# sanazkaviani/3d-latent-diffusion-model

Hardware: AMD Instinct MI355X
Metric: UNet denoising steps/sec (bf16, 1x4x24x24x24 latent; whole job = sum over GPUs) (higher is better)
Workload: dtype bf16

## Files before the change

3d-latent-diffusion-model_amd/csrc/attention.h:

```cpp
#pragma once
#include "common.h"

struct AttnParams {
    const bf16_t* qkv; bf16_t* out;
    int B, N, C, heads; float scale;
    float* lse;
    int d;
};

template <int S, int QW, bool DB, int D = 64>
__global__ __launch_bounds__(64 * QW * S) void attn_fwd_kernel(const AttnParams p) {
    constexpr int KT = 64;
    constexpr int NSL = (D + 63) / 64, DS = D < 64 ? D : 64;
    constexpr int K2 = DS / 32, NDT = DS / 16, CH = DS / 8;
    constexpr int IMG = KT * 128;
    constexpr int TILE = 2 * NSL * IMG;
    constexpr int GT = 64 * QW;
    constexpr int NIT = (KT * CH * NSL) / GT;
    static_assert(S == 1 || D == 64, "the in-workgroup key split is built for D = 64");
    static_assert((KT * CH * NSL) % GT == 0, "staging must divide evenly");
    extern __shared__ __attribute__((aligned(16))) char smem_all[];

    const int tid = threadIdx.x % GT, lane = tid & 63, wave = tid >> 6, grp = threadIdx.x / GT;
    char* smem = smem_all + grp * (DB ? 2 : 1) * TILE;
    const int fr = lane & 15, fg = lane >> 4;
    const int b = blockIdx.z, head = blockIdx.y;
    const int q0 = blockIdx.x * (16 * QW) + wave * 16;
    const int ld = 3 * p.C;
    const bf16_t* base = p.qkv + (size_t)b * p.N * ld;
    const int hoff = head * D;

    bf16x8 qf[NSL][K2];
    {
        int qr = q0 + fr; if (qr >= p.N) qr = p.N - 1;
#pragma unroll
        for (int sl = 0; sl < NSL; ++sl)
#pragma unroll
            for (int k2 = 0; k2 < K2; ++k2)
                qf[sl][k2] = *reinterpret_cast<const bf16x8*>(base + (size_t)qr * ld + hoff + sl * 64 + k2 * 32 + 8 * fg);
    }

    f32x4 ot[NSL][NDT];
#pragma unroll
    for (int sl = 0; sl < NSL; ++sl)
#pragma unroll
        for (int i = 0; i < NDT; ++i) ot[sl][i] = (f32x4){0.f, 0.f, 0.f, 0.f};
    float mrun = -INFINITY, lrun = 0.f;
    const float cexp = p.scale * 1.44269504088896340736f;

    u32x4 kreg[NIT], vreg[NIT];
    auto stage_load = [&](int k0) {
#pragma unroll
        for (int it = 0; it < NIT; ++it) {
            const int idx = tid + it * GT;
            const int sl = idx / (KT * CH), rem = idx - sl * (KT * CH);
            const int row = rem / CH, ch = rem - row * CH;
            int kr = k0 + row; if (kr >= p.N) kr = p.N - 1;
            const bf16_t* tok = base + (size_t)kr * ld + hoff + sl * 64 + ch * 8;
            kreg[it] = *reinterpret_cast<const u32x4*>(tok + p.C);
            vreg[it] = *reinterpret_cast<const u32x4*>(tok + 2 * p.C);
        }
    };
    auto stage_write = [&](char* ks, char* vs) {
#pragma unroll
        for (int it = 0; it < NIT; ++it) {
            const int idx = tid + it * GT;
            const int sl = idx / (KT * CH), rem = idx - sl * (KT * CH);
            const int row = rem / CH, ch = rem - row * CH;
            *reinterpret_cast<u32x4*>(ks + sl * IMG + row * 128 + ((ch ^ ((row >> 1) & 7)) << 4)) = kreg[it];
            *reinterpret_cast<u32x4*>(vs + sl * IMG + row * 128 + ((ch ^ (((row >> 1) & 3) << 1)) << 4)) = vreg[it];
        }
    };

    const int ntile = (p.N + KT - 1) / KT;
    const int nrounds = (ntile + S - 1) / S;
    stage_load(grp * KT);
#pragma unroll
    for (int sl = 0; sl < NSL; ++sl)
#pragma unroll
        for (int k2 = 0; k2 < K2; ++k2) asm volatile("" :: "v"(qf[sl][k2]));
    stage_write(smem, smem + NSL * IMG);
    __syncthreads();
    for (int it = 0; it < nrounds; ++it) {
        const int t = it * S + grp;
        const int k0 = t * KT;
        const char* ks = smem + (DB ? (it & 1) * TILE : 0);
        const char* vs = ks + NSL * IMG;
        stage_load(k0 + S * KT);
        if (t < ntile) {
        f32x4 st[4];
#pragma unroll
        for (int j = 0; j < 4; ++j) {
            st[j] = (f32x4){0.f, 0.f, 0.f, 0.f};
            const int row = j * 16 + fr;
#pragma unroll
            for (int sl = 0; sl < NSL; ++sl)
#pragma unroll
                for (int k2 = 0; k2 < K2; ++k2) {
                    const int c = k2 * 4 + fg;
                    const bf16x8 kf = *reinterpret_cast<const bf16x8*>(ks + sl * IMG + row * 128 + ((c ^ ((row >> 1) & 7)) << 4));
                    st[j] = __builtin_amdgcn_mfma_f32_16x16x32_bf16(kf, qf[sl][k2], st[j], 0, 0, 0);
                }
        }
        if (k0 + KT > p.N) {
#pragma unroll
            for (int j = 0; j < 4; ++j)
#pragma unroll
                for (int r = 0; r < 4; ++r)
                    if (k0 + 16 * j + 4 * fg + r >= p.N) st[j][r] = -INFINITY;
        }
        float tmax = fmaxf(fmaxf(fmaxf(st[0][0], st[0][1]), fmaxf(st[0][2], st[0][3])), fmaxf(fmaxf(st[1][0], st[1][1]), fmaxf(st[1][2], st[1][3])));
        tmax = fmaxf(tmax, fmaxf(fmaxf(fmaxf(st[2][0], st[2][1]), fmaxf(st[2][2], st[2][3])), fmaxf(fmaxf(st[3][0], st[3][1]), fmaxf(st[3][2], st[3][3]))));
        tmax = fmaxf(tmax, __shfl_xor(tmax, 16, 64));
        tmax = fmaxf(tmax, __shfl_xor(tmax, 32, 64));
        const float mnew = fmaxf(mrun, tmax);
        const float alpha = __builtin_amdgcn_exp2f((mrun - mnew) * cexp);
        const float mc = -mnew * cexp;
        mrun = mnew;
        float psum = 0.f;
        bf16x8 pf[2];
#pragma unroll
        for (int h = 0; h < 2; ++h) {
            float pv[8];
#pragma unroll
            for (int e = 0; e < 8; ++e) {
                const float pe = __builtin_amdgcn_exp2f(fmaf(st[2 * h + (e >> 2)][e & 3], cexp, mc));
                psum += pe;
                pv[e] = pe;
            }
            u32x4 pk;
#pragma unroll
            for (int e = 0; e < 4; ++e) pk[e] = pack2bf(pv[2 * e], pv[2 * e + 1]);
            pf[h] = *reinterpret_cast<bf16x8*>(&pk);
        }
        lrun = lrun * alpha + psum;
        if (__builtin_amdgcn_ballot_w64(alpha != 1.0f)) {
#pragma unroll
            for (int sl = 0; sl < NSL; ++sl)
#pragma unroll
                for (int dt = 0; dt < NDT; ++dt) {
#pragma unroll
                    for (int r = 0; r < 4; ++r) ot[sl][dt][r] *= alpha;
                }
        }
        typedef __attribute__((ext_vector_type(4))) short s16x4;
        typedef __attribute__((address_space(3))) s16x4* lds_s16x4_t;
        const int tq = fr >> 2, tp = fr & 3;
#pragma unroll
        for (int sl = 0; sl < NSL; ++sl)
#pragma unroll
        for (int dt = 0; dt < NDT; ++dt) {
#pragma unroll
            for (int h = 0; h < 2; ++h) {
                const int rlo = (2 * h) * 16 + 4 * fg + tq, rhi = rlo + 16;
                const char* alo = vs + sl * IMG + rlo * 128 + ((dt ^ ((rlo >> 1) & 3)) << 5) + tp * 8;
                const char* ahi = vs + sl * IMG + rhi * 128 + ((dt ^ ((rhi >> 1) & 3)) << 5) + tp * 8;
                const s16x4 lo = __builtin_amdgcn_ds_read_tr16_b64_v4i16((lds_s16x4_t)alo);
                const s16x4 hi = __builtin_amdgcn_ds_read_tr16_b64_v4i16((lds_s16x4_t)ahi);
                const bf16x8 vf = {lo[0], lo[1], lo[2], lo[3], hi[0], hi[1], hi[2], hi[3]};
                ot[sl][dt] = __builtin_amdgcn_mfma_f32_16x16x32_bf16(vf, pf[h], ot[sl][dt], 0, 0, 0);
            }
        }
        }
        if constexpr (!DB) __syncthreads();
        {
            char* nk = smem + (DB ? ((it + 1) & 1) * TILE : 0);
            stage_write(nk, nk + NSL * IMG);
        }
        __syncthreads();
    }
    lrun += __shfl_xor(lrun, 16, 64);
    lrun += __shfl_xor(lrun, 32, 64);
    if constexpr (S > 1) {
        float* xo = reinterpret_cast<float*>(smem_all) + (size_t)(grp * QW + wave) * (1024 + 32);
        if (grp > 0) {
#pragma unroll
            for (int dt = 0; dt < NDT; ++dt) *reinterpret_cast<f32x4*>(xo + (dt * 64 + lane) * 4) = ot[0][dt];
            if (fg == 0) { xo[1024 + fr] = mrun; xo[1040 + fr] = lrun; }
        }
        __syncthreads();
        if (grp > 0) return;
#pragma unroll
        for (int g = 1; g < S; ++g) {
            const float* xg = reinterpret_cast<const float*>(smem_all) + (size_t)(g * QW + wave) * (1024 + 32);
            const float mg = xg[1024 + fr], lg = xg[1040 + fr];
            const float mnew = fmaxf(mrun, mg);
            const float a0 = __builtin_amdgcn_exp2f((mrun - mnew) * cexp), a1 = __builtin_amdgcn_exp2f((mg - mnew) * cexp);
            lrun = lrun * a0 + lg * a1;
            mrun = mnew;
#pragma unroll
            for (int dt = 0; dt < NDT; ++dt) {
                const f32x4 og = *reinterpret_cast<const f32x4*>(xg + (dt * 64 + lane) * 4);
#pragma unroll
                for (int r = 0; r < 4; ++r) ot[0][dt][r] = ot[0][dt][r] * a0 + og[r] * a1;
            }
        }
    }
    const float inv = 1.0f / lrun;
    const int qr = q0 + fr;
    if (p.lse && qr < p.N && fg == 0) p.lse[((size_t)b * p.heads + head) * p.N + qr] = mrun * p.scale + __logf(lrun);
    if (qr < p.N) {
        bf16_t* orow = p.out + ((size_t)b * p.N + qr) * p.C + hoff;
#pragma unroll
        for (int sl = 0; sl < NSL; ++sl)
#pragma unroll
        for (int dt = 0; dt < NDT; ++dt) {
            u32x2 o;
            o[0] = pack2bf(ot[sl][dt][0] * inv, ot[sl][dt][1] * inv);
            o[1] = pack2bf(ot[sl][dt][2] * inv, ot[sl][dt][3] * inv);
            *reinterpret_cast<u32x2*>(orow + sl * 64 + dt * 16 + 4 * fg) = o;
        }
    }
}

template <int D>
static inline hipError_t launch_attn_fwd_d(const AttnParams& p, hipStream_t s) {
    constexpr int LDS = 2 * 2 * ((D + 63) / 64) * 64 * 128;
    static bool once_tab[32] = {}; bool& once = attr_flag(once_tab);
    if (!once) {
        hipError_t e = hipFuncSetAttribute(reinterpret_cast<const void*>(&attn_fwd_kernel<1, 4, true, D>), hipFuncAttributeMaxDynamicSharedMemorySize, LDS);
        if (e != hipSuccess) return e;
        once = true;
    }
    hipLaunchKernelGGL((attn_fwd_kernel<1, 4, true, D>), dim3((p.N + 63) / 64, p.heads, p.B), dim3(256), LDS, s, p);
    return hipGetLastError();
}
static inline hipError_t launch_attn_fwd(const AttnParams& p, hipStream_t s) {
    if (p.d == 32) return launch_attn_fwd_d<32>(p, s);
    if (p.d == 128) return launch_attn_fwd_d<128>(p, s);
    if (p.d == 256) return launch_attn_fwd_d<256>(p, s);
    if (p.d != 64) return hipErrorInvalidValue;
    static bool once_tab[32] = {}; bool& once = attr_flag(once_tab);
    if (!once) {
        hipError_t e = hipFuncSetAttribute(reinterpret_cast<const void*>(&attn_fwd_kernel<4, 4, true>), hipFuncAttributeMaxDynamicSharedMemorySize, 4 * 32768);
        if (e == hipSuccess) e = hipFuncSetAttribute(reinterpret_cast<const void*>(&attn_fwd_kernel<8, 2, false>), hipFuncAttributeMaxDynamicSharedMemorySize, 8 * 16384);
        if (e != hipSuccess) return e;
        once = true;
    }
    if (p.N >= 1024 && (long)((p.N + 63) / 64) * p.heads * p.B < 128)
        hipLaunchKernelGGL((attn_fwd_kernel<8, 2, false>), dim3((p.N + 31) / 32, p.heads, p.B), dim3(1024), 8 * 16384, s, p);
    else if (p.N > 3 * 64) hipLaunchKernelGGL((attn_fwd_kernel<4, 4, true>), dim3((p.N + 63) / 64, p.heads, p.B), dim3(1024), 4 * 32768, s, p);
    else hipLaunchKernelGGL((attn_fwd_kernel<1, 4, true>), dim3((p.N + 63) / 64, p.heads, p.B), dim3(256), 32768, s, p);
    return hipGetLastError();
}


struct AttnBwdParams {
    const bf16_t* qkv; const bf16_t* o; const bf16_t* d_o; const float* lse;
    float* delta;
    bf16_t* dqkv;
    int B, N, C, heads; float scale;
    int d;
};

__global__ __launch_bounds__(256) void attn_delta_kernel(const AttnBwdParams p) {
    const long idx = (long)blockIdx.x * 256 + threadIdx.x;
    const int cpd = p.d >> 3;
    const long total = (long)p.B * p.N * p.heads * cpd;
    float s = 0.f;
    long tok = 0; int head = 0;
    if (idx < total) {
        const int ch = (int)(idx % cpd);
        const long th = idx / cpd;
        head = (int)(th % p.heads); tok = th / p.heads;
        const u32x4 a = *reinterpret_cast<const u32x4*>(p.o + tok * p.C + head * p.d + ch * 8);
        const u32x4 b = *reinterpret_cast<const u32x4*>(p.d_o + tok * p.C + head * p.d + ch * 8);
#pragma unroll
        for (int k = 0; k < 4; ++k)
            s += __uint_as_float(a[k] << 16) * __uint_as_float(b[k] << 16) +
                 __uint_as_float(a[k] & 0xffff0000u) * __uint_as_float(b[k] & 0xffff0000u);
    }
    for (int o = 1; o < cpd; o <<= 1) s += __shfl_xor(s, o, 64);
    if (idx < total && (idx % cpd) == 0) {
        const long bb = tok / p.N, i = tok - bb * p.N;
        p.delta[((size_t)bb * p.heads + head) * p.N + i] = s;
    }
}

typedef __attribute__((ext_vector_type(4))) short attn_s16x4;
typedef __attribute__((address_space(3))) attn_s16x4* attn_lds_s16x4_t;

__device__ __forceinline__ int attn_row_off(int row, int ch) { return row * 128 + ((ch ^ ((row >> 1) & 7)) << 4); }
__device__ __forceinline__ int attn_tr_off(int row, int ch) { return row * 128 + ((ch ^ (((row >> 1) & 3) << 1)) << 4); }
__device__ __forceinline__ bf16x8 attn_tr_frag(const char* img, int dt, int h, int fr, int fg) {
    const int tq = fr >> 2, tp = fr & 3;
    const int rlo = (2 * h) * 16 + 4 * fg + tq, rhi = rlo + 16;
    const attn_s16x4 lo = __builtin_amdgcn_ds_read_tr16_b64_v4i16((attn_lds_s16x4_t)(img + rlo * 128 + ((dt ^ ((rlo >> 1) & 3)) << 5) + tp * 8));
    const attn_s16x4 hi = __builtin_amdgcn_ds_read_tr16_b64_v4i16((attn_lds_s16x4_t)(img + rhi * 128 + ((dt ^ ((rhi >> 1) & 3)) << 5) + tp * 8));
    return (bf16x8){lo[0], lo[1], lo[2], lo[3], hi[0], hi[1], hi[2], hi[3]};
}

template <int D>
__global__ __launch_bounds__(256) void attn_bwd_dq_kernel(const AttnBwdParams p) {
    constexpr int KT = 64;
    constexpr int NSL = (D + 63) / 64, DS = D < 64 ? D : 64, K2 = DS / 32, NDT = DS / 16, CH = DS / 8, IMG = KT * 128;
    constexpr int NIT = (KT * CH * NSL) / 256;
    extern __shared__ __attribute__((aligned(16))) char smem[];
    char* k_row = smem; char* k_tr = smem + NSL * IMG; char* v_row = smem + 2 * NSL * IMG;
    const int tid = threadIdx.x, lane = tid & 63, wave = tid >> 6;
    const int fr = lane & 15, fg = lane >> 4;
    const int b = blockIdx.z, head = blockIdx.y;
    const int q0 = blockIdx.x * 64 + wave * 16;
    const int ld = 3 * p.C, hoff = head * D;
    const bf16_t* base = p.qkv + (size_t)b * p.N * ld;
    int qr = q0 + fr; const bool qok = qr < p.N; if (!qok) qr = p.N - 1;
    bf16x8 qf[NSL][K2], dof[NSL][K2];
#pragma unroll
    for (int sl = 0; sl < NSL; ++sl)
#pragma unroll
    for (int k2 = 0; k2 < K2; ++k2) {
        qf[sl][k2] = *reinterpret_cast<const bf16x8*>(base + (size_t)qr * ld + hoff + sl * 64 + k2 * 32 + 8 * fg);
        dof[sl][k2] = *reinterpret_cast<const bf16x8*>(p.d_o + ((size_t)b * p.N + qr) * p.C + hoff + sl * 64 + k2 * 32 + 8 * fg);
    }
    const float lse = p.lse[((size_t)b * p.heads + head) * p.N + qr];
    const float dlt = p.delta[((size_t)b * p.heads + head) * p.N + qr];
    f32x4 dq[NSL][NDT];
#pragma unroll
    for (int sl = 0; sl < NSL; ++sl)
#pragma unroll
    for (int i = 0; i < NDT; ++i) dq[sl][i] = (f32x4){0.f, 0.f, 0.f, 0.f};
    const int ntile = (p.N + KT - 1) / KT;
    u32x4 kreg[NIT], vreg[NIT];
    auto stage_load = [&](int k0) {
#pragma unroll
        for (int it = 0; it < NIT; ++it) {
            const int idx = tid + it * 256, sl = idx / (KT * CH), rem = idx - sl * (KT * CH), row = rem / CH, ch = rem - row * CH;
            int kr = k0 + row; if (kr >= p.N) kr = p.N - 1;
            const bf16_t* tok = base + (size_t)kr * ld + hoff + sl * 64 + ch * 8;
            kreg[it] = *reinterpret_cast<const u32x4*>(tok + p.C);
            vreg[it] = *reinterpret_cast<const u32x4*>(tok + 2 * p.C);
        }
    };
    stage_load(0);
#pragma unroll
    for (int sl = 0; sl < NSL; ++sl)
#pragma unroll
        for (int k2 = 0; k2 < K2; ++k2) asm volatile("" :: "v"(qf[sl][k2]), "v"(dof[sl][k2]));
    asm volatile("" :: "v"(lse), "v"(dlt));
    for (int t = 0; t < ntile; ++t) {
        const int k0 = t * KT;
        __syncthreads();
#pragma unroll
        for (int it = 0; it < NIT; ++it) {
            const int idx = tid + it * 256, sl = idx / (KT * CH), rem = idx - sl * (KT * CH), row = rem / CH, ch = rem - row * CH;
            *reinterpret_cast<u32x4*>(k_row + sl * IMG + attn_row_off(row, ch)) = kreg[it];
            *reinterpret_cast<u32x4*>(k_tr + sl * IMG + attn_tr_off(row, ch)) = kreg[it];
            *reinterpret_cast<u32x4*>(v_row + sl * IMG + attn_row_off(row, ch)) = vreg[it];
        }
        __syncthreads();
        stage_load(k0 + KT);
        bf16x8 dsf[2];
        f32x4 st[4], dp[4];
#pragma unroll
        for (int j = 0; j < 4; ++j) {
            st[j] = (f32x4){0.f, 0.f, 0.f, 0.f}; dp[j] = (f32x4){0.f, 0.f, 0.f, 0.f};
            const int row = j * 16 + fr;
#pragma unroll
            for (int sl = 0; sl < NSL; ++sl)
#pragma unroll
            for (int k2 = 0; k2 < K2; ++k2) {
                const bf16x8 kf = *reinterpret_cast<const bf16x8*>(k_row + sl * IMG + attn_row_off(row, k2 * 4 + fg));
                const bf16x8 vf = *reinterpret_cast<const bf16x8*>(v_row + sl * IMG + attn_row_off(row, k2 * 4 + fg));
                st[j] = __builtin_amdgcn_mfma_f32_16x16x32_bf16(kf, qf[sl][k2], st[j], 0, 0, 0);
                dp[j] = __builtin_amdgcn_mfma_f32_16x16x32_bf16(vf, dof[sl][k2], dp[j], 0, 0, 0);
            }
        }
#pragma unroll
        for (int h = 0; h < 2; ++h) {
            float dsv[8];
#pragma unroll
            for (int e = 0; e < 8; ++e) {
                const int j = 2 * h + (e >> 2), r = e & 3;
                const int key = k0 + 16 * j + 4 * fg + r;
                const float pe = (key < p.N) ? __expf(st[j][r] * p.scale - lse) : 0.f;
                dsv[e] = pe * (dp[j][r] - dlt);
            }
            u32x4 pk;
#pragma unroll
            for (int e = 0; e < 4; ++e) pk[e] = pack2bf(dsv[2 * e], dsv[2 * e + 1]);
            dsf[h] = *reinterpret_cast<bf16x8*>(&pk);
        }
#pragma unroll
        for (int sl = 0; sl < NSL; ++sl)
#pragma unroll
        for (int dt = 0; dt < NDT; ++dt)
#pragma unroll
            for (int h = 0; h < 2; ++h)
                dq[sl][dt] = __builtin_amdgcn_mfma_f32_16x16x32_bf16(attn_tr_frag(k_tr + sl * IMG, dt, h, fr, fg), dsf[h], dq[sl][dt], 0, 0, 0);
    }
    if (qok) {
        bf16_t* orow = p.dqkv + ((size_t)b * p.N + qr) * ld + hoff;
#pragma unroll
        for (int sl = 0; sl < NSL; ++sl)
#pragma unroll
        for (int dt = 0; dt < NDT; ++dt) {
            u32x2 o;
            o[0] = pack2bf(dq[sl][dt][0] * p.scale, dq[sl][dt][1] * p.scale);
            o[1] = pack2bf(dq[sl][dt][2] * p.scale, dq[sl][dt][3] * p.scale);
            *reinterpret_cast<u32x2*>(orow + sl * 64 + dt * 16 + 4 * fg) = o;
        }
    }
}

template <int D>
__global__ __launch_bounds__(256) void attn_bwd_dkv_kernel(const AttnBwdParams p) {
    constexpr int QT = 64;
    constexpr int NSL = (D + 63) / 64, DS = D < 64 ? D : 64, K2 = DS / 32, NDT = DS / 16, CH = DS / 8, IMG = QT * 128;
    constexpr int NIT = (QT * CH * NSL) / 256;
    extern __shared__ __attribute__((aligned(16))) char smem[];
    char* q_row = smem; char* q_tr = smem + NSL * IMG; char* do_row = smem + 2 * NSL * IMG; char* do_tr = smem + 3 * NSL * IMG;
    float* s_lse = reinterpret_cast<float*>(smem + 4 * NSL * IMG); float* s_dlt = s_lse + QT;
    const int tid = threadIdx.x, lane = tid & 63, wave = tid >> 6;
    const int fr = lane & 15, fg = lane >> 4;
    const int b = blockIdx.z, head = blockIdx.y;
    const int kv0 = blockIdx.x * 64 + wave * 16;
    const int ld = 3 * p.C, hoff = head * D;
    const bf16_t* base = p.qkv + (size_t)b * p.N * ld;
    int kr = kv0 + fr; const bool kok = kr < p.N; if (!kok) kr = p.N - 1;
    bf16x8 kf[NSL][K2], vf[NSL][K2];
#pragma unroll
    for (int sl = 0; sl < NSL; ++sl)
#pragma unroll
    for (int k2 = 0; k2 < K2; ++k2) {
        kf[sl][k2] = *reinterpret_cast<const bf16x8*>(base + (size_t)kr * ld + p.C + hoff + sl * 64 + k2 * 32 + 8 * fg);
        vf[sl][k2] = *reinterpret_cast<const bf16x8*>(base + (size_t)kr * ld + 2 * p.C + hoff + sl * 64 + k2 * 32 + 8 * fg);
    }
    f32x4 dk[NSL][NDT], dv[NSL][NDT];
#pragma unroll
    for (int sl = 0; sl < NSL; ++sl)
#pragma unroll
    for (int i = 0; i < NDT; ++i) { dk[sl][i] = (f32x4){0.f, 0.f, 0.f, 0.f}; dv[sl][i] = (f32x4){0.f, 0.f, 0.f, 0.f}; }
    const int ntile = (p.N + QT - 1) / QT;
    u32x4 qreg[NIT], oreg[NIT]; float lreg = 0.f, dreg = 0.f;
    auto stage_load = [&](int q0) {
#pragma unroll
        for (int it = 0; it < NIT; ++it) {
            const int idx = tid + it * 256, sl = idx / (QT * CH), rem = idx - sl * (QT * CH), row = rem / CH, ch = rem - row * CH;
            int qr = q0 + row; if (qr >= p.N) qr = p.N - 1;
            qreg[it] = *reinterpret_cast<const u32x4*>(base + (size_t)qr * ld + hoff + sl * 64 + ch * 8);
            oreg[it] = *reinterpret_cast<const u32x4*>(p.d_o + ((size_t)b * p.N + qr) * p.C + hoff + sl * 64 + ch * 8);
        }
        {
            int qr = q0 + (tid & (QT - 1)); const bool ok = qr < p.N; if (!ok) qr = p.N - 1;
            const float l = p.lse[((size_t)b * p.heads + head) * p.N + qr];
            lreg = ok ? l : INFINITY;
            dreg = p.delta[((size_t)b * p.heads + head) * p.N + qr];
        }
    };
    stage_load(0);
#pragma unroll
    for (int sl = 0; sl < NSL; ++sl)
#pragma unroll
        for (int k2 = 0; k2 < K2; ++k2) asm volatile("" :: "v"(kf[sl][k2]), "v"(vf[sl][k2]));
    for (int t = 0; t < ntile; ++t) {
        const int q0 = t * QT;
        __syncthreads();
#pragma unroll
        for (int it = 0; it < NIT; ++it) {
            const int idx = tid + it * 256, sl = idx / (QT * CH), rem = idx - sl * (QT * CH), row = rem / CH, ch = rem - row * CH;
            *reinterpret_cast<u32x4*>(q_row + sl * IMG + attn_row_off(row, ch)) = qreg[it];
            *reinterpret_cast<u32x4*>(q_tr + sl * IMG + attn_tr_off(row, ch)) = qreg[it];
            *reinterpret_cast<u32x4*>(do_row + sl * IMG + attn_row_off(row, ch)) = oreg[it];
            *reinterpret_cast<u32x4*>(do_tr + sl * IMG + attn_tr_off(row, ch)) = oreg[it];
        }
        if (tid < QT) { s_lse[tid] = lreg; s_dlt[tid] = dreg; }
        __syncthreads();
        stage_load(q0 + QT);
        f32x4 st[4], dp[4];
#pragma unroll
        for (int j = 0; j < 4; ++j) {
            st[j] = (f32x4){0.f, 0.f, 0.f, 0.f}; dp[j] = (f32x4){0.f, 0.f, 0.f, 0.f};
            const int row = j * 16 + fr;
#pragma unroll
            for (int sl = 0; sl < NSL; ++sl)
#pragma unroll
            for (int k2 = 0; k2 < K2; ++k2) {
                const bf16x8 qf = *reinterpret_cast<const bf16x8*>(q_row + sl * IMG + attn_row_off(row, k2 * 4 + fg));
                const bf16x8 of = *reinterpret_cast<const bf16x8*>(do_row + sl * IMG + attn_row_off(row, k2 * 4 + fg));
                st[j] = __builtin_amdgcn_mfma_f32_16x16x32_bf16(qf, kf[sl][k2], st[j], 0, 0, 0);
                dp[j] = __builtin_amdgcn_mfma_f32_16x16x32_bf16(of, vf[sl][k2], dp[j], 0, 0, 0);
            }
        }
        bf16x8 pf[2], dsf[2];
#pragma unroll
        for (int h = 0; h < 2; ++h) {
            float pv[8], dsv[8];
#pragma unroll
            for (int e = 0; e < 8; ++e) {
                const int j = 2 * h + (e >> 2), r = e & 3;
                const int ql = 16 * j + 4 * fg + r;
                const float pe = __expf(st[j][r] * p.scale - s_lse[ql]);
                pv[e] = pe; dsv[e] = pe * (dp[j][r] - s_dlt[ql]);
            }
            u32x4 pk, dk_;
#pragma unroll
            for (int e = 0; e < 4; ++e) { pk[e] = pack2bf(pv[2 * e], pv[2 * e + 1]); dk_[e] = pack2bf(dsv[2 * e], dsv[2 * e + 1]); }
            pf[h] = *reinterpret_cast<bf16x8*>(&pk); dsf[h] = *reinterpret_cast<bf16x8*>(&dk_);
        }
#pragma unroll
        for (int sl = 0; sl < NSL; ++sl)
#pragma unroll
        for (int dt = 0; dt < NDT; ++dt)
#pragma unroll
            for (int h = 0; h < 2; ++h) {
                dv[sl][dt] = __builtin_amdgcn_mfma_f32_16x16x32_bf16(attn_tr_frag(do_tr + sl * IMG, dt, h, fr, fg), pf[h], dv[sl][dt], 0, 0, 0);
                dk[sl][dt] = __builtin_amdgcn_mfma_f32_16x16x32_bf16(attn_tr_frag(q_tr + sl * IMG, dt, h, fr, fg), dsf[h], dk[sl][dt], 0, 0, 0);
            }
    }
    if (kok) {
        bf16_t* orow = p.dqkv + ((size_t)b * p.N + kr) * ld + hoff;
#pragma unroll
        for (int sl = 0; sl < NSL; ++sl)
#pragma unroll
        for (int dt = 0; dt < NDT; ++dt) {
            u32x2 o;
            o[0] = pack2bf(dk[sl][dt][0] * p.scale, dk[sl][dt][1] * p.scale); o[1] = pack2bf(dk[sl][dt][2] * p.scale, dk[sl][dt][3] * p.scale);
            *reinterpret_cast<u32x2*>(orow + p.C + sl * 64 + dt * 16 + 4 * fg) = o;
            o[0] = pack2bf(dv[sl][dt][0], dv[sl][dt][1]); o[1] = pack2bf(dv[sl][dt][2], dv[sl][dt][3]);
            *reinterpret_cast<u32x2*>(orow + 2 * p.C + sl * 64 + dt * 16 + 4 * fg) = o;
        }
    }
}

template <int D>
static inline hipError_t launch_attn_bwd_d(const AttnBwdParams& p, hipStream_t s) {
    constexpr int NSL = (D + 63) / 64;
    constexpr int LDS_DQ = 3 * NSL * 64 * 128, LDS_DKV = 4 * NSL * 64 * 128 + 2 * 64 * 4;
    static bool once_tab[32] = {}; bool& once = attr_flag(once_tab);
    if (!once) {
        hipError_t e = hipFuncSetAttribute(reinterpret_cast<const void*>(&attn_bwd_dq_kernel<D>), hipFuncAttributeMaxDynamicSharedMemorySize, LDS_DQ);
        if (e == hipSuccess) e = hipFuncSetAttribute(reinterpret_cast<const void*>(&attn_bwd_dkv_kernel<D>), hipFuncAttributeMaxDynamicSharedMemorySize, LDS_DKV);
        if (e != hipSuccess) return e;
        once = true;
    }
    const long dthreads = (long)p.B * p.N * p.heads * (D / 8);
    hipLaunchKernelGGL(attn_delta_kernel, dim3((unsigned)((dthreads + 255) / 256)), dim3(256), 0, s, p);
    hipLaunchKernelGGL(attn_bwd_dq_kernel<D>, dim3((p.N + 63) / 64, p.heads, p.B), dim3(256), LDS_DQ, s, p);
    hipLaunchKernelGGL(attn_bwd_dkv_kernel<D>, dim3((p.N + 63) / 64, p.heads, p.B), dim3(256), LDS_DKV, s, p);
    return hipGetLastError();
}
static inline hipError_t launch_attn_bwd(const AttnBwdParams& p, hipStream_t s) {
    switch (p.d) {
        case 32: return launch_attn_bwd_d<32>(p, s);
        case 64: return launch_attn_bwd_d<64>(p, s);
// ... 6 lines not shown
```

3d-latent-diffusion-model_amd/csrc/common.h:

```cpp
#pragma once
#include <stdlib.h>
#include <hip/hip_runtime.h>
#include <stdint.h>

typedef uint16_t bf16_t;
typedef __attribute__((ext_vector_type(8))) short bf16x8;
typedef __attribute__((ext_vector_type(4))) float f32x4;
typedef __attribute__((ext_vector_type(4))) unsigned int u32x4;
typedef __attribute__((ext_vector_type(2))) unsigned int u32x2;

#define LDM_WAVE 64

static inline bool& attr_flag(bool (&tab)[32]) { int d = 0; if (hipGetDevice(&d) != hipSuccess || d < 0 || d >= 32) d = 0; return tab[d]; }

__device__ __forceinline__ float bf2f(bf16_t v) { return __uint_as_float(((uint32_t)v) << 16); }

__device__ __forceinline__ bf16_t f2bf(float f) {
    __bf16 b = (__bf16)f;
    return *reinterpret_cast<bf16_t*>(&b);
}
__device__ __forceinline__ uint32_t pack2bf(float lo, float hi) {
    return (uint32_t)f2bf(lo) | ((uint32_t)f2bf(hi) << 16);
}
__device__ __forceinline__ float silu_f(float x) { return x / (1.0f + __expf(-x)); }

static inline long ldm_knob(const char* name, long dflt) { const char* e = getenv(name); return (e && *e) ? atol(e) : dflt; }
#ifdef LDM_EXPERIMENTS
static inline long ldm_xknob(const char* name, long dflt) { return ldm_knob(name, dflt); }
#else
static inline long ldm_xknob(const char*, long dflt) { return dflt; }
#endif

template <bool WT>
__device__ __forceinline__ void store16(void* ptr, u32x4 v) {
    if constexpr (WT) asm volatile("global_store_dwordx4 %0, %1, off sc1\n\ts_nop 1" ::"v"(ptr), "v"(v) : "memory");
    else *reinterpret_cast<u32x4*>(ptr) = v;
}

__device__ __forceinline__ float wave_sum(float v) {
#pragma unroll
    for (int o = 32; o > 0; o >>= 1) v += __shfl_xor(v, o, 64);
    return v;
}

#ifdef LDM_KSTAMPS
#ifndef LDM_KSTAMP_BLOCK
#define LDM_KSTAMP_BLOCK 0
#endif
__device__ unsigned long long g_kstamp[8192 * 8];
__device__ unsigned g_kstamp_seq;
struct KStamp {
    unsigned slot;
    __device__ __forceinline__ KStamp(int id) {
        slot = 0xffffffffu;
        if (blockIdx.x == LDM_KSTAMP_BLOCK && (blockIdx.y | blockIdx.z) == 0 && threadIdx.x == 0) {
            const unsigned long long t = __builtin_amdgcn_s_memrealtime();
            slot = atomicAdd(&g_kstamp_seq, 1u) & 8191u;
            g_kstamp[slot * 8] = (unsigned long long)id; g_kstamp[slot * 8 + 1] = t;
            for (int k = 2; k < 8; ++k) g_kstamp[slot * 8 + k] = 0;
        }
    }
    __device__ __forceinline__ void at(int k) { if (slot != 0xffffffffu) g_kstamp[slot * 8 + 1 + k] = __builtin_amdgcn_s_memrealtime(); }
};
#define KSTAMP_BEGIN(id) KStamp kst_(id)
#define KSTAMP(k) kst_.at(k)
#define KSTAMP_DRAIN(k) do { asm volatile("s_waitcnt vmcnt(0) lgkmcnt(0)" ::: "memory"); kst_.at(k); } while (0)
#define KSTAMP_PARAM , KStamp& kst_
#define KSTAMP_ARG , kst_
#else
#define KSTAMP_PARAM
#define KSTAMP_ARG
#define KSTAMP_BEGIN(id) do { } while (0)
#define KSTAMP(k) do { } while (0)
#define KSTAMP_DRAIN(k) do { } while (0)
#endif
```

3d-latent-diffusion-model_amd/csrc/conv_igemm.h:

```cpp
#pragma once
#include "common.h"

struct ConvParams {
    const bf16_t* x0a; const bf16_t* x0b; int c0a, c0b;
    const bf16_t* w0;
    const bf16_t* x1a; const bf16_t* x1b; int c1a, c1b;
    const bf16_t* w1;
    const bf16_t* zero_page;
    int N, Din, Hin, Win;
    int Dout, Hout, Wout;
    int ksize, stride, pad, ups;
    int exact;
    int M;
    int CoutS;
    int CoutPad;
    int CoutReal;
    int nchunk0, nchunk1;
    int steps0, steps1;
    int splitk, steps_per_split;
    int mtiles, ntiles;
    int halo_mtps, q_per_split;
    int tile_order;
    int phase_mode, mtiles_pp;
    int x3_n;
    int raw_partial;
    unsigned fd_hw_m, fd_hw_s, fd_w_m, fd_w_s;
    int slab_lg;
    float* out32; const float* residual32;
    const float* bias;
    const float* bias2;
    const float* temb; int temb_stride;
    const bf16_t* residual;
    bf16_t* out;
    float* out_f32;
    float* partial;
    float* stats;
    unsigned long long* stamps;
    int dbg;
};

__device__ __forceinline__ float* slab_ptr(float* partial, int split, int M, int CoutPad, int lg, int m, int c) {
    float* base = partial + (size_t)split * M * CoutPad;
    if (lg == 0) return base + (size_t)m * CoutPad + c;
    return base + (((size_t)(c >> lg) * M + m) << lg) + (c & ((1 << lg) - 1));
}


static inline void fastdiv_make(unsigned d, unsigned* m, unsigned* s) {
    if (d <= 1) { *m = 0; *s = 255u; return; }
    unsigned l = 0; while ((1ull << l) < d) ++l;
    *m = (unsigned)((((1ull << l) - d) << 32) / d + 1); *s = l - 1;
}
__device__ __forceinline__ unsigned fastdiv(unsigned n, unsigned m, unsigned s) {
    if (s == 255u) return n;
    const unsigned q = __umulhi(n, m);
    return (((n - q) >> 1) + q) >> s;
}

__device__ __forceinline__ int xcd_remap(int bid, int nwg) {
    int q = nwg >> 3, r = nwg & 7, x = bid & 7, i = bid >> 3;
    int base = (x < r) ? x * (q + 1) : r * (q + 1) + (x - r) * q;
    return base + i;
}

__device__ __forceinline__ void glds16(const void* gsrc, void* lds_dst) {
    __builtin_amdgcn_global_load_lds((const __attribute__((address_space(1))) void*)gsrc,
                                     (__attribute__((address_space(3))) void*)lds_dst, 16, 0, 0);
}

template <int WGM, int WGN, int BK, int NS, int NG>
__global__ __launch_bounds__(256 * NG, 2) void conv_igemm_kernel(const ConvParams p) {
#if defined(__HIP_DEVICE_COMPILE__)
    constexpr int BM = 64 * WGM, BN = 64 * WGN;
    constexpr int RB = BK * 2;
    constexpr int CPR = RB / 16;
    constexpr int RPP = 1024 / RB;
    constexpr int NW = 4 * NG;
    constexpr int PA = BM / RPP / NW;
    constexpr int PB = BN / RPP / NW;
    constexpr int STAGE = (BM + BN) * RB;
    constexpr int SWZ_SHIFT = (CPR == 8) ? 1 : 2;
    constexpr int KS = BK / 32;
    constexpr int PF = NS - 1;
    constexpr int LPS = PA + PB;
    static_assert(PA >= 1 && PB >= 1, "tile too small for this many waves");
    static_assert(KS == NG, "each wave group computes exactly one 32-deep k-substep per K step");
    static_assert((PF - 1) * LPS <= 63 && PF * LPS <= 63, "vmcnt is a 6-bit counter");
    static_assert(NG == 1 || NS * STAGE >= 65536 + 4 * BN * 8, "the accumulator exchange needs 64 KiB of LDS (+ the GroupNorm fold)");
    static_assert(NS * STAGE + 28 * BM * 4 <= 160 * 1024, "ring + tap table must fit the 160 KiB LDS");
    extern __shared__ __attribute__((aligned(16))) char smem[];
    typedef __attribute__((address_space(3))) void* lds_ptr_t;

    KSTAMP_BEGIN(7);
    const int tid = threadIdx.x;
    const int lane = tid & 63;
    const int wave = __builtin_amdgcn_readfirstlane(tid >> 6);
    const int grp = wave >> 2;
    const int wq = wave & 3;
    const int wm = wq % WGM, wn = wq / WGM;

    const int nwg = gridDim.x;
    int lid = xcd_remap(blockIdx.x, nwg);
    int mtile, ntile, split;
    if (p.tile_order == 1) {
        ntile = lid % p.ntiles; lid /= p.ntiles; mtile = lid % p.mtiles; split = lid / p.mtiles;
    } else {
        mtile = lid % p.mtiles; lid /= p.mtiles; ntile = lid % p.ntiles; split = lid / p.ntiles;
    }
    int m0 = mtile * BM; const int n0 = ntile * BN;
    int Mloc = p.M;
    int ph_n = 0, ph_d = 0, ph_h = 0, ph_w = 0;
    const bf16_t* w0p = p.w0;
    if (p.phase_mode) {
        const int t8 = mtile / p.mtiles_pp, phase = t8 & 7;
        m0 = (mtile - t8 * p.mtiles_pp) * BM; ph_n = t8 >> 3;
        ph_d = phase >> 2; ph_h = (phase >> 1) & 1; ph_w = phase & 1;
        Mloc = p.Din * p.Hin * p.Win;
        w0p += (size_t)phase * 8 * p.CoutPad * (p.c0a + p.c0b);
    }
    const int steps_total = p.steps0 + p.steps1;
    const int s_begin = split * p.steps_per_split;
    int s_end = s_begin + p.steps_per_split; if (s_end > steps_total) s_end = steps_total;
    const int nsteps = s_end - s_begin;
    const int dbg = p.dbg;
    if (dbg & 128) return;
#define LDM_STAMP(I) do { if ((dbg & 512) && tid == 0) p.stamps[(size_t)blockIdx.x * 8 + (I)] = __builtin_amdgcn_s_memrealtime(); } while (0)
    LDM_STAMP(0);

    const int prow = lane / CPR;
    const int pchunk = lane % CPR;
    const int DHWo = p.Dout * p.Hout * p.Wout;
    const int HWo = p.Hout * p.Wout;
    const int DinU = p.Din << p.ups, HinU = p.Hin << p.ups, WinU = p.Win << p.ups;
    const int rows_in0 = p.N * p.Din * p.Hin * p.Win;

    int* const tapv = reinterpret_cast<int*>(smem + NS * STAGE);
    {
        constexpr int TPR = (256 * NG) / BM;
        const int row = tid / TPR, part = tid % TPR;
        const int m = m0 + row;
        const int taps = p.ksize * p.ksize * p.ksize;
        if (row < BM) {
            int n = 0, od = 0, oh = 0, ow = 0;
            if (p.phase_mode) {
                n = ph_n;
                if (m < Mloc) { od = m / (p.Hin * p.Win); int r = m - od * p.Hin * p.Win; oh = r / p.Win; ow = r - oh * p.Win; }
            } else if (m < p.M) { n = m / DHWo; int r = m - n * DHWo; od = r / HWo; r -= od * HWo; oh = r / p.Wout; ow = r - oh * p.Wout; }
            const int nb = n * p.Din * p.Hin * p.Win;
            if (part == 0) tapv[taps * BM + row] = -1;
            if (p.phase_mode) {
                for (int tap = part; tap < 8; tap += TPR) {
                    const int id = od + (tap >> 2) - 1 + ph_d, ih = oh + ((tap >> 1) & 1) - 1 + ph_h, iw = ow + (tap & 1) - 1 + ph_w;
                    const bool ok = (m < Mloc) & ((unsigned)id < (unsigned)p.Din) & ((unsigned)ih < (unsigned)p.Hin) &
                                    ((unsigned)iw < (unsigned)p.Win) & !(dbg & 1);
                    tapv[tap * BM + row] = ok ? nb + (id * p.Hin + ih) * p.Win + iw : -1;
                }
            } else
            for (int tap = part; tap < taps; tap += TPR) {
                int kd = 0, kh = 0, kw = 0;
                if (p.ksize == 3) { kd = tap / 9; kh = (tap - kd * 9) / 3; kw = tap - kd * 9 - kh * 3; }
                const int id = od * p.stride + kd - p.pad, ih = oh * p.stride + kh - p.pad, iw = ow * p.stride + kw - p.pad;
                const bool ok = (m < Mloc) & ((unsigned)id < (unsigned)DinU) & ((unsigned)ih < (unsigned)HinU) &
                                ((unsigned)iw < (unsigned)WinU) & !(dbg & 1) & !(p.exact & (id | ih | iw) & 1);
                tapv[tap * BM + row] = ok ? nb + ((id >> p.ups) * p.Hin + (ih >> p.ups)) * p.Win + (iw >> p.ups) : -1;
            }
        }
    }
    int a_row[PA], a_m[PA], a_kb[PA];
#pragma unroll
    for (int j = 0; j < PA; ++j) {
        const int row = (wave * PA + j) * RPP + prow;
        const int swz = (row >> SWZ_SHIFT) & (CPR - 1);
        a_kb[j] = (pchunk ^ swz) * 16;
        a_row[j] = row;
        a_m[j] = (m0 + row < Mloc && !(dbg & 1)) ? m0 + row : -1;
    }
    int b_row[PB], b_kb[PB];
#pragma unroll
    for (int j = 0; j < PB; ++j) {
        const int R = (wave * PB + j) * RPP + prow;
        const int swz = (R >> SWZ_SHIFT) & (CPR - 1);
        b_kb[j] = (pchunk ^ swz) * 16;
        const int q = R >> 6, nt = (R >> 4) & 3, i = R & 15;
        b_row[j] = ((dbg & 2) ? 0 : n0 + 64 * q + 16 * (i >> 2) + 4 * nt + (i & 3));
    }

    const unsigned x3s2 = p.x3_n ? (unsigned)p.x3_n * 256u : 0u;
    int sg_grp, sg_tap, sg_src, sg_left;
    int g_ca = 0, g_cb = 0;
    unsigned g_wtap = 0;
    unsigned soff_a = 0, soff_b = 0;
    int a_v[PA];
    unsigned a_vo[PA], b_vo[PB];
    __amdgpu_buffer_rsrc_t rs_a, rs_a0, rs_a1, rs_b;
    int ld_s = s_begin;
    int first_cis;
    {
        int chunk;
        if (ld_s < p.steps0) {
            sg_grp = 0; sg_tap = ld_s / p.nchunk0; chunk = ld_s - sg_tap * p.nchunk0;
        } else { sg_grp = 1; sg_tap = 0; chunk = ld_s - p.steps0; }
        const int ca = sg_grp ? p.c1a : p.c0a;
        sg_src = (chunk * BK >= ca) ? 1 : 0;
        first_cis = sg_src ? chunk - ca / BK : chunk;
        sg_left = -1;
    }

#define LDM_GROUP_SETUP() do {                                                                                \
        g_ca = sg_grp ? p.c1a : p.c0a; g_cb = sg_grp ? p.c1b : p.c0b;                                         \
        const int cin_ = g_ca + g_cb;                                                                         \
        const unsigned rows_ = sg_grp ? (unsigned)p.M : (unsigned)rows_in0;                                   \
        rs_a0 = __builtin_amdgcn_make_buffer_rsrc((void*)(sg_grp ? p.x1a : p.x0a), 0, (int)(rows_ * (x3s2 ? x3s2 : (unsigned)g_ca * 2u)), 0x00020000); \
        rs_a1 = __builtin_amdgcn_make_buffer_rsrc((void*)(sg_grp ? p.x1b : p.x0b), 0, (int)(rows_ * (x3s2 ? x3s2 : (unsigned)g_cb * 2u)), 0x00020000); \
        g_wtap = (unsigned)p.CoutPad * (unsigned)cin_ * 2u;                                                   \
        rs_b = __builtin_amdgcn_make_buffer_rsrc((void*)(sg_grp ? p.w1 : w0p), 0,                            \
                                                 (int)((unsigned)(sg_grp ? 1 : p.ksize * p.ksize * p.ksize) * g_wtap), 0x00020000); \
        _Pragma("unroll") for (int j = 0; j < PB; ++j)                                                        \
            b_vo[j] = (unsigned)b_row[j] * (unsigned)(cin_ * 2) + (unsigned)b_kb[j];                          \
    } while (0)
#define LDM_TAP_SETUP() do {                                                                                  \
        _Pragma("unroll") for (int j = 0; j < PA; ++j)                                                        \
            a_v[j] = (sg_grp == 0) ? tapv[sg_tap * BM + a_row[j]] : a_m[j];                                   \
    } while (0)
#define LDM_SRC_SETUP() do {                                                                                  \
        const unsigned cs2_ = x3s2 ? x3s2 : (unsigned)(sg_src ? g_cb : g_ca) * 2u;    \
        rs_a = sg_src ? rs_a1 : rs_a0;                                                                        \
        _Pragma("unroll") for (int j = 0; j < PA; ++j)                                                        \
            a_vo[j] = (a_v[j] >= 0) ? (unsigned)a_v[j] * cs2_ + (unsigned)a_kb[j] : 0xFFFFFFFFu;              \
    } while (0)
#define LDM_SEG_ADVANCE() do {                                                                                \
        if (sg_left <= 0) {                                                                                   \
            if (sg_left < 0) {                                              \
                LDM_GROUP_SETUP(); LDM_TAP_SETUP(); LDM_SRC_SETUP();                                          \
                soff_a = (unsigned)first_cis * (BK * 2);                                                      \
                soff_b = (unsigned)sg_tap * g_wtap + (unsigned)((sg_src ? g_ca : 0) + first_cis * BK) * 2u;   \
                sg_left = (sg_src ? g_cb : g_ca) / BK - first_cis;                                            \
            } else if (sg_src == 0 && g_cb > 0) {                          \
                sg_src = 1; LDM_SRC_SETUP();                                                                  \
                soff_a = 0; sg_left = g_cb / BK;                              \
            } else {                                                    \
                sg_src = 0;                                                                                   \
                if (sg_grp == 0 && ld_s >= p.steps0) { sg_grp = 1; sg_tap = 0; LDM_GROUP_SETUP(); }           \
                else ++sg_tap;                                                                                  \
                LDM_TAP_SETUP(); LDM_SRC_SETUP();                                                             \
                soff_a = 0; soff_b = (unsigned)sg_tap * g_wtap; sg_left = g_ca / BK;                          \
            }                                                                                                 \
        }                                                                                                     \
    } while (0)
#define LDM_DMA_RAW() do {                                                                                    \
        {                                                                                                     \
            char* st_ = smem + ((ld_s - s_begin) % NS) * STAGE;                                               \
            _Pragma("unroll") for (int j = 0; j < PA; ++j)                                                    \
                __builtin_amdgcn_raw_ptr_buffer_load_lds(rs_a, (lds_ptr_t)(st_ + (wave * PA + j) * 1024), 16, \
                                                         a_vo[j], soff_a, 0, 0);                              \
            _Pragma("unroll") for (int j = 0; j < PB; ++j)                                                    \
                __builtin_amdgcn_raw_ptr_buffer_load_lds(rs_b, (lds_ptr_t)(st_ + BM * RB + (wave * PB + j) * 1024), \
                                                         16, b_vo[j], soff_b, 0, 0);                          \
        }                                                                                                     \
        soff_a += BK * 2; soff_b += BK * 2; --sg_left; ++ld_s;                                                \
    } while (0)
#define LDM_DMA() do {                                                                                        \
        if (!(dbg & 4)) LDM_DMA_RAW();                                                                        \
        else { soff_a += BK * 2; soff_b += BK * 2; --sg_left; ++ld_s; }                                       \
    } while (0)
#define LDM_ISSUE() do { LDM_SEG_ADVANCE(); LDM_DMA(); } while (0)

    const int fr = lane & 15, fg = lane >> 4;
    const int ra0 = wm * 64 + fr, rb0 = wn * 64 + fr;
    const int cfrag = grp * 4 + fg;
    const int a_rd0 = ra0 * RB + ((cfrag ^ ((ra0 >> SWZ_SHIFT) & (CPR - 1))) << 4);
    const int b_rd0 = BM * RB + rb0 * RB + ((cfrag ^ ((rb0 >> SWZ_SHIFT) & (CPR - 1))) << 4);

    f32x4 acc[4][4];
#pragma unroll
    for (int a = 0; a < 4; ++a)
#pragma unroll
        for (int b = 0; b < 4; ++b) acc[a][b] = (f32x4){0.f, 0.f, 0.f, 0.f};

    bf16x8 wfA[4], afA[4], wfB[4], afB[4];

#define LDM_READ_FRAGS_RAW(WF, AF, SLOT) do {                                                       \
        {                                                                                           \
            const char* sb_ = smem + (SLOT) * STAGE;                                                \
            _Pragma("unroll") for (int t = 0; t < 4; ++t) {                                         \
                WF[t] = *reinterpret_cast<const bf16x8*>(sb_ + b_rd0 + t * 16 * RB);                \
                AF[t] = *reinterpret_cast<const bf16x8*>(sb_ + a_rd0 + t * 16 * RB);                \
            }                                                                                       \
        }                                                                                           \
    } while (0)
#define LDM_READ_FRAGS(WF, AF, SLOT) do { if (!(dbg & 16)) LDM_READ_FRAGS_RAW(WF, AF, SLOT); } while (0)
#define LDM_MFMA16_RAW(WF, AF) do {                                                                 \
        {                                                                                           \
            _Pragma("unroll") for (int nt = 0; nt < 4; ++nt)                                        \
                _Pragma("unroll") for (int mt = 0; mt < 4; ++mt)                                    \
                    acc[nt][mt] = __builtin_amdgcn_mfma_f32_16x16x32_bf16(WF[nt], AF[mt], acc[nt][mt], 0, 0, 0); \
        }                                                                                           \
    } while (0)
#define LDM_MFMA16(WF, AF) do { if (!(dbg & 8)) LDM_MFMA16_RAW(WF, AF); } while (0)
#define LDM_NEXT_STEP_READY(S) do {                                                                 \
        if ((S) + PF < s_end) asm volatile("s_waitcnt vmcnt(%0)" ::"n"((PF - 1) * LPS) : "memory"); \
        else asm volatile("s_waitcnt vmcnt(0)" ::: "memory");                                       \
        __builtin_amdgcn_s_barrier();                                                               \
        asm volatile("" ::: "memory");                                                              \
    } while (0)
#define LDM_HALF(S, WC, AC, WN, AN) do {                                                            \
        LDM_ST2(S, 0);                                                                              \
        __builtin_amdgcn_s_waitcnt(0xC07F);                                                         \
        if ((S) + 1 < s_end) {                                                                      \
            LDM_NEXT_STEP_READY(S);                                                                 \
            if (grp == 0 && ld_s < s_end) LDM_ISSUE();                                              \
            LDM_READ_FRAGS(WN, AN, ((S) + 1 - s_begin) % NS);                                       \
        }                                                                                           \
        LDM_MFMA16(WC, AC);                                                                         \
        if (grp == 1 && (S) + 1 < s_end && ld_s < s_end) LDM_ISSUE();                              \
    } while (0)

    LDM_STAMP(1);
    KSTAMP(1);
    if (dbg & 256) return;
    __syncthreads();
    if (nsteps > 0) {
#pragma unroll
        for (int i = 0; i < NS; ++i) if (i < nsteps) LDM_ISSUE();
        if (nsteps > PF) asm volatile("s_waitcnt vmcnt(%0)" ::"n"(PF * LPS) : "memory");
        else asm volatile("s_waitcnt vmcnt(0)" ::: "memory");
        __builtin_amdgcn_s_barrier();
        asm volatile("" ::: "memory");
        LDM_READ_FRAGS(wfA, afA, 0);
    }
    LDM_STAMP(2);
    KSTAMP(2);
#define LDM_ST2(S, K) do { if ((dbg & 1024) && tid == 0 && (S) - s_begin < 120) p.stamps[(size_t)gridDim.x * 8 + (size_t)blockIdx.x * 512 + ((S) - s_begin) * 4 + (K)] = __builtin_amdgcn_s_memrealtime(); } while (0)
#define LDM_FAST_TAIL(WC, AC, WN, AN, S) \
        LDM_READ_FRAGS_RAW(WN, AN, ((S) + 1 - s_begin) % NS);                                       \
        LDM_MFMA16_RAW(WC, AC);                                                                     \
        _Pragma("unroll") for (int i_ = 0; i_ < LPS; ++i_) {                                        \
            __builtin_amdgcn_sched_group_barrier(0x008, 1, 0);                          \
            __builtin_amdgcn_sched_group_barrier(0x004, 2, 0);                \
            __builtin_amdgcn_sched_group_barrier(0x020, 1, 0);      \
        }                                                                                           \
        _Pragma("unroll") for (int i_ = 0; i_ < 8; ++i_) {                                          \
            __builtin_amdgcn_sched_group_barrier(0x008, 1, 0);                          \
            __builtin_amdgcn_sched_group_barrier(0x100, 1, 0);                  \
        }                                                                                           \
        __builtin_amdgcn_sched_group_barrier(0x008, 16 - LPS - 8 > 0 ? 16 - LPS - 8 : 0, 0);
#define LDM_FAST_SYNC(S) \
        __builtin_amdgcn_s_waitcnt(0xC07F);                                                         \
        asm volatile("s_waitcnt vmcnt(%0)" ::"n"((PF - 1) * LPS) : "memory");                       \
        LDM_ST2(S, 2);                                                                              \
        __builtin_amdgcn_s_barrier();                                                               \
        asm volatile("" ::: "memory");                                                              \
        LDM_ST2(S, 3);
#define LDM_FAST_COPIES() \
            char* st_ = smem + ((ld_s - s_begin) % NS) * STAGE;                                     \
            _Pragma("unroll") for (int j = 0; j < PA; ++j)                                          \
                __builtin_amdgcn_raw_ptr_buffer_load_lds(rs_a, (lds_ptr_t)(st_ + (wave * PA + j) * 1024), 16, \
                                                         a_vo[j], soff_a, 0, 0);                    \
            _Pragma("unroll") for (int j = 0; j < PB; ++j)                                          \
                __builtin_amdgcn_raw_ptr_buffer_load_lds(rs_b, (lds_ptr_t)(st_ + BM * RB + (wave * PB + j) * 1024), \
                                                         16, b_vo[j], soff_b, 0, 0);
#define LDM_FAST_HALF(S, WC, AC, WN, AN) do {                                                       \
        LDM_ST2(S, 0);                                                                              \
        LDM_FAST_SYNC(S)                                                                            \
        {                                                                                           \
            LDM_FAST_COPIES()                                                                       \
// ... 356 lines not shown
```

Before: 526.1.

## Add two-deep K/V prefetch attention variant with XCD remap for long sequences

For long-sequence, low-block-count attention, the launch switches from the 8-way key split with 1024 threads to a 4-way split with 512 threads. The new variant keeps two register sets of K/V tiles in flight to hide global-load latency, uses 24-bit multiply offsets, and packs bf16 with a vector convert. It also remaps block IDs across XCDs for L2 locality. The cost is more registers for the deeper prefetch and fewer threads per block, which may reduce latency hiding if occupancy drops.

```diff
diff --git a/3d-latent-diffusion-model_amd/csrc/attention.h b/3d-latent-diffusion-model_amd/csrc/attention.h
--- a/3d-latent-diffusion-model_amd/csrc/attention.h
+++ b/3d-latent-diffusion-model_amd/csrc/attention.h
@@ -1,5 +1,12 @@
 #pragma once
 #include "common.h"
+
+__device__ __forceinline__ uint32_t pack2bf_pk(float lo, float hi) {
+    typedef __attribute__((ext_vector_type(2))) float attn_f32x2;
+    typedef __attribute__((ext_vector_type(2))) __bf16 attn_bf16x2;
+    const attn_bf16x2 b = __builtin_convertvector((attn_f32x2){lo, hi}, attn_bf16x2);
+    return *reinterpret_cast<const uint32_t*>(&b);
+}
 
 struct AttnParams {
     const bf16_t* qkv; bf16_t* out;
@@ -8,7 +15,7 @@
     int d;
 };
 
-template <int S, int QW, bool DB, int D = 64>
+template <int S, int QW, bool DB, int D = 64, int PF = 1, bool XR = false>
 __global__ __launch_bounds__(64 * QW * S) void attn_fwd_kernel(const AttnParams p) {
     constexpr int KT = 64;
     constexpr int NSL = (D + 63) / 64, DS = D < 64 ? D : 64;
@@ -24,8 +31,12 @@
     const int tid = threadIdx.x % GT, lane = tid & 63, wave = tid >> 6, grp = threadIdx.x / GT;
     char* smem = smem_all + grp * (DB ? 2 : 1) * TILE;
     const int fr = lane & 15, fg = lane >> 4;
-    const int b = blockIdx.z, head = blockIdx.y;
-    const int q0 = blockIdx.x * (16 * QW) + wave * 16;
+    int b = blockIdx.z, head = blockIdx.y, qblk = blockIdx.x;
+    if constexpr (XR) {
+        const int lid = xcd_remap((int)(blockIdx.x + gridDim.x * (blockIdx.y + gridDim.y * blockIdx.z)), (int)(gridDim.x * gridDim.y * gridDim.z));
+        qblk = lid % (int)gridDim.x; head = (lid / (int)gridDim.x) % (int)gridDim.y; b = lid / (int)(gridDim.x * gridDim.y);
+    }
+    const int q0 = qblk * (16 * QW) + wave * 16;
     const int ld = 3 * p.C;
     const bf16_t* base = p.qkv + (size_t)b * p.N * ld;
     const int hoff = head * D;
@@ -48,45 +59,52 @@
     float mrun = -INFINITY, lrun = 0.f;
     const float cexp = p.scale * 1.44269504088896340736f;
 
-    u32x4 kreg[NIT], vreg[NIT];
-    auto stage_load = [&](int k0) {
+    u32x4 kreg[PF][NIT], vreg[PF][NIT];
+    auto stage_load = [&](int set, int k0) {
 #pragma unroll
         for (int it = 0; it < NIT; ++it) {
             const int idx = tid + it * GT;
             const int sl = idx / (KT * CH), rem = idx - sl * (KT * CH);
             const int row = rem / CH, ch = rem - row * CH;
             int kr = k0 + row; if (kr >= p.N) kr = p.N - 1;
+            if constexpr (PF > 1) {
+                const unsigned off = __umul24((unsigned)kr, (unsigned)(2 * ld)) + (unsigned)(2 * (p.C + hoff + sl * 64 + ch * 8));
+                kreg[set][it] = *reinterpret_cast<const u32x4*>(reinterpret_cast<const char*>(base) + off);
+                vreg[set][it] = *reinterpret_cast<const u32x4*>(reinterpret_cast<const char*>(base) + (off + 2u * p.C));
+            } else {
             const bf16_t* tok = base + (size_t)kr * ld + hoff + sl * 64 + ch * 8;
-            kreg[it] = *reinterpret_cast<const u32x4*>(tok + p.C);
-            vreg[it] = *reinterpret_cast<const u32x4*>(tok + 2 * p.C);
+            kreg[set][it] = *reinterpret_cast<const u32x4*>(tok + p.C);
+            vreg[set][it] = *reinterpret_cast<const u32x4*>(tok + 2 * p.C);
+            }
         }
     };
-    auto stage_write = [&](char* ks, char* vs) {
+    auto stage_write = [&](int set, char* ks, char* vs) {
 #pragma unroll
         for (int it = 0; it < NIT; ++it) {
             const int idx = tid + it * GT;
             const int sl = idx / (KT * CH), rem = idx - sl * (KT * CH);
             const int row = rem / CH, ch = rem - row * CH;
-            *reinterpret_cast<u32x4*>(ks + sl * IMG + row * 128 + ((ch ^ ((row >> 1) & 7)) << 4)) = kreg[it];
-            *reinterpret_cast<u32x4*>(vs + sl * IMG + row * 128 + ((ch ^ (((row >> 1) & 3) << 1)) << 4)) = vreg[it];
+            *reinterpret_cast<u32x4*>(ks + sl * IMG + row * 128 + ((ch ^ ((row >> 1) & 7)) << 4)) = kreg[set][it];
+            *reinterpret_cast<u32x4*>(vs + sl * IMG + row * 128 + ((ch ^ (((row >> 1) & 3) << 1)) << 4)) = vreg[set][it];
         }
     };
 
     const int ntile = (p.N + KT - 1) / KT;
     const int nrounds = (ntile + S - 1) / S;
-    stage_load(grp * KT);
+#pragma unroll
+    for (int u = 0; u < PF; ++u) stage_load(u, (grp + u * S) * KT);
 #pragma unroll
     for (int sl = 0; sl < NSL; ++sl)
 #pragma unroll
         for (int k2 = 0; k2 < K2; ++k2) asm volatile("" :: "v"(qf[sl][k2]));
-    stage_write(smem, smem + NSL * IMG);
+    stage_write(0, smem, smem + NSL * IMG);
     __syncthreads();
-    for (int it = 0; it < nrounds; ++it) {
+    auto round = [&](const int it, const int u, const bool MAIN) __attribute__((always_inline)) {
         const int t = it * S + grp;
         const int k0 = t * KT;
         const char* ks = smem + (DB ? (it & 1) * TILE : 0);
         const char* vs = ks + NSL * IMG;
-        stage_load(k0 + S * KT);
+        if (MAIN) stage_load(u, k0 + PF * S * KT);
         if (t < ntile) {
         f32x4 st[4];
 #pragma unroll
@@ -130,7 +148,7 @@
             }
             u32x4 pk;
 #pragma unroll
-            for (int e = 0; e < 4; ++e) pk[e] = pack2bf(pv[2 * e], pv[2 * e + 1]);
+            for (int e = 0; e < 4; ++e) pk[e] = PF > 1 ? pack2bf_pk(pv[2 * e], pv[2 * e + 1]) : pack2bf(pv[2 * e], pv[2 * e + 1]);
             pf[h] = *reinterpret_cast<bf16x8*>(&pk);
         }
         lrun = lrun * alpha + psum;
@@ -163,12 +181,19 @@
         }
         }
         if constexpr (!DB) __syncthreads();
-        {
+        if (MAIN || it + 1 < nrounds) {
             char* nk = smem + (DB ? ((it + 1) & 1) * TILE : 0);
-            stage_write(nk, nk + NSL * IMG);
+            stage_write((u + 1) % PF, nk, nk + NSL * IMG);
         }
         __syncthreads();
-    }
+    };
+    const int nmain = nrounds - nrounds % PF;
+    for (int it0 = 0; it0 < nmain; it0 += PF)
+#pragma unroll
+        for (int u = 0; u < PF; ++u) round(it0 + u, u, true);
+#pragma unroll
+    for (int u = 0; u + 1 < PF; ++u)
+        if (nmain + u < nrounds) round(nmain + u, u, false);
     lrun += __shfl_xor(lrun, 16, 64);
     lrun += __shfl_xor(lrun, 32, 64);
     if constexpr (S > 1) {
@@ -234,12 +259,18 @@
     if (!once) {
         hipError_t e = hipFuncSetAttribute(reinterpret_cast<const void*>(&attn_fwd_kernel<4, 4, true>), hipFuncAttributeMaxDynamicSharedMemorySize, 4 * 32768);
         if (e == hipSuccess) e = hipFuncSetAttribute(reinterpret_cast<const void*>(&attn_fwd_kernel<8, 2, false>), hipFuncAttributeMaxDynamicSharedMemorySize, 8 * 16384);
+        if (e == hipSuccess) e = hipFuncSetAttribute(reinterpret_cast<const void*>(&attn_fwd_kernel<4, 2, true, 64, 2>), hipFuncAttributeMaxDynamicSharedMemorySize, 4 * 32768);
+        if (e == hipSuccess) e = hipFuncSetAttribute(reinterpret_cast<const void*>(&attn_fwd_kernel<4, 2, true, 64, 2, true>), hipFuncAttributeMaxDynamicSharedMemorySize, 4 * 32768);
         if (e != hipSuccess) return e;
         once = true;
     }
-    if (p.N >= 1024 && (long)((p.N + 63) / 64) * p.heads * p.B < 128)
-        hipLaunchKernelGGL((attn_fwd_kernel<8, 2, false>), dim3((p.N + 31) / 32, p.heads, p.B), dim3(1024), 8 * 16384, s, p);
-    else if (p.N > 3 * 64) hipLaunchKernelGGL((attn_fwd_kernel<4, 4, true>), dim3((p.N + 63) / 64, p.heads, p.B), dim3(1024), 4 * 32768, s, p);
+    static const bool attn_long = ldm_knob("LDM_ATTN_LONG", 1) != 0;
+    static const bool attn_xcd = ldm_knob("LDM_ATTN_XCD", 1) != 0;
+    if (p.N >= 1024 && (long)((p.N + 63) / 64) * p.heads * p.B < 128) {
+        if (attn_long && attn_xcd) hipLaunchKernelGGL((attn_fwd_kernel<4, 2, true, 64, 2, true>), dim3((p.N + 31) / 32, p.heads, p.B), dim3(512), 4 * 32768, s, p);
+        else if (attn_long) hipLaunchKernelGGL((attn_fwd_kernel<4, 2, true, 64, 2>), dim3((p.N + 31) / 32, p.heads, p.B), dim3(512), 4 * 32768, s, p);
+        else hipLaunchKernelGGL((attn_fwd_kernel<8, 2, false>), dim3((p.N + 31) / 32, p.heads, p.B), dim3(1024), 8 * 16384, s, p);
+    } else if (p.N > 3 * 64) hipLaunchKernelGGL((attn_fwd_kernel<4, 4, true>), dim3((p.N + 63) / 64, p.heads, p.B), dim3(1024), 4 * 32768, s, p);
     else hipLaunchKernelGGL((attn_fwd_kernel<1, 4, true>), dim3((p.N + 63) / 64, p.heads, p.B), dim3(256), 32768, s, p);
     return hipGetLastError();
 }
diff --git a/3d-latent-diffusion-model_amd/csrc/common.h b/3d-latent-diffusion-model_amd/csrc/common.h
--- a/3d-latent-diffusion-model_amd/csrc/common.h
+++ b/3d-latent-diffusion-model_amd/csrc/common.h
@@ -37,6 +37,12 @@
     else *reinterpret_cast<u32x4*>(ptr) = v;
 }
 
+__device__ __forceinline__ int xcd_remap(int bid, int nwg) {
+    int q = nwg >> 3, r = nwg & 7, x = bid & 7, i = bid >> 3;
+    int base = (x < r) ? x * (q + 1) : r * (q + 1) + (x - r) * q;
+    return base + i;
+}
+
 __device__ __forceinline__ float wave_sum(float v) {
 #pragma unroll
     for (int o = 32; o > 0; o >>= 1) v += __shfl_xor(v, o, 64);
diff --git a/3d-latent-diffusion-model_amd/csrc/conv_igemm.h b/3d-latent-diffusion-model_amd/csrc/conv_igemm.h
--- a/3d-latent-diffusion-model_amd/csrc/conv_igemm.h
+++ b/3d-latent-diffusion-model_amd/csrc/conv_igemm.h
@@ -55,12 +55,6 @@
     if (s == 255u) return n;
     const unsigned q = __umulhi(n, m);
     return (((n - q) >> 1) + q) >> s;
-}
-
-__device__ __forceinline__ int xcd_remap(int bid, int nwg) {
-    int q = nwg >> 3, r = nwg & 7, x = bid & 7, i = bid >> 3;
-    int base = (x < r) ? x * (q + 1) : r * (q + 1) + (x - r) * q;
-    return base + i;
 }
 
 __device__ __forceinline__ void glds16(const void* gsrc, void* lds_dst) {
```

New measurement: 533.2, median of 6. +1.4%, better.
